# cocowy1/Cost-Volume-Aggregation-in-Stereo-Matching-Revisited

Hardware: AMD Instinct MI355X
Metric: cost-volumes/sec (fwd+bwd) at 544x960 D=192 (higher is better)
Workload: dtype f32

## Files before the change

### cost-volume-aggregation-in-stereo-matching-revisited_amd/csrc/conv3d_wgrad_s2_f16x2.hip

```cpp
#include "dca_frag.h"
#include <type_traits>

namespace {

constexpr int NT = 2;
constexpr int TH = 4, TW = 16;
constexpr int NROW = TH;
constexpr int FD = 3, FH = 2 * TH + 1, NFROW = FD * FH;
constexpr int FV = 2 * TW + 1;
constexpr int VB = 64;
constexpr int X_TERM = NFROW * FV * VB;
constexpr int Y_BLK = NROW * TW * VB;
constexpr int Y_TERM = 2 * Y_BLK;
constexpr int X_OFF = 0, Y_OFF = NT * X_TERM;
constexpr int LDS_BYTES = Y_OFF + NT * Y_TERM;
constexpr int NXQ = NFROW * 8 * 4;
constexpr int KXQ = (NXQ + 511) / 512;
constexpr int NXE = NFROW * 4;
constexpr int NYQ = 2 * NROW * 4 * 4;
static_assert(NXQ - 512 + NYQ <= 512, "coarse items fit behind the second round of fine items");

struct WS2Args {
  const float* x;
  const float* dy;
  float* part;
  int N, Cx, Cy, D, H, W;
  int Do, Ho, Wo;
  int nTD, nTH, nTW, nCxT, nCyP;
  const int* xexps;
  const int* yexps;
};

__global__ __launch_bounds__(512) void wgrad3s2_f16x2_kernel(WS2Args a) {
  extern __shared__ __attribute__((aligned(16))) char smem[];
  const int tid = threadIdx.x, lane = tid & 63, wv = tid >> 6, l31 = lane & 31, half = lane >> 5;
  const int blk = wv >> 2, wq = wv & 3;
  const int ct = blockIdx.y, cyp = ct / a.nCxT, cx0 = (ct % a.nCxT) * 32, cy0 = cyp * 64;
  const bool blk_on = cy0 + 32 * blk < a.Cy;

  const long T = (long)a.N * a.nTD * a.nTH * a.nTW;
  const int nx = gridDim.x >= 8 ? 8 : 1, xcd = blockIdx.x % nx;
  const int cnt = (gridDim.x - xcd + nx - 1) / nx;
  const int t_begin = (int)(T * xcd / nx) + blockIdx.x / nx, t_end = (int)(T * (xcd + 1) / nx), t_step = cnt;

  f32x16 acc[7];
#pragma unroll
  for (int j = 0; j < 7; ++j)
#pragma unroll
    for (int r = 0; r < 16; ++r) acc[j][r] = 0.f;

  const int cstride = a.D * a.H * a.W, ystride = a.Do * a.Ho * a.Wo;
  const long xsample = (long)a.Cx * cstride, ysample = (long)a.Cy * ystride;

  const int q4 = (lane & 15) >> 2, chb = (16 * ((lane >> 4) & 1) + 4 * (lane & 3)) * 2;
  const int lane_off_x = (2 * (8 * half + q4)) * VB + chb;
  const int lane_off_y = (8 * half + q4) * VB + chb;

  float4 rq[KXQ][8];
  float re[8];
  int* ex_lds = (int*)(smem + LDS_BYTES);
  if (tid < 32) ex_lds[tid] = (cx0 + tid < a.Cx) ? dca_coherent_loadi(a.xexps + cx0 + tid) : 0;
  else if (tid < 96) ex_lds[tid] = (cy0 + tid - 32 < a.Cy) ? dca_coherent_loadi(a.yexps + cy0 + tid - 32) : 0;
  __syncthreads();
  const int yu = tid - (NXQ - 512);
  auto decode = [&](int tile, int& n, int& d0, int& h0, int& w0) __attribute__((always_inline)) {
    const int tw = tile % a.nTW; tile /= a.nTW;
    const int th = tile % a.nTH; tile /= a.nTH;
    const int td = tile % a.nTD;
    n = tile / a.nTD;
    d0 = td; h0 = th * TH; w0 = tw * TW;
  };
  auto load_tile = [&](int n, int d0, int h0, int w0, int part = -1) __attribute__((always_inline)) {
    const __amdgpu_buffer_rsrc_t xr = dca_rsrc(a.x + (long)n * xsample, xsample * 4);
    const __amdgpu_buffer_rsrc_t yr = dca_rsrc(a.dy + (long)n * ysample, ysample * 4);
#pragma unroll
    for (int k = 0; k < KXQ; ++k) {
      if ((part == 0 && k >= 1) || (part == 1 && k < 1)) continue;
      const int it = tid + 512 * k, cg = it & 3, quad = (it >> 2) & 7, frow = it >> 5;
      const int d = 2 * d0 - 1 + frow / FH, h = 2 * h0 - 1 + frow % FH, w = 2 * w0 + 4 * quad, c0 = cx0 + cg * 8;
      const int ok = (int)(it < NXQ) & (int)((unsigned)d < (unsigned)a.D) & (int)((unsigned)h < (unsigned)a.H) & (int)(w + 3 < a.W);
      const int off = (c0 * cstride + (d * a.H + h) * a.W + w) * 4;
      if (512 * k + (tid & ~63) < NXQ) {
#pragma unroll
        for (int j = 0; j < 8; ++j) rq[k][j] = dca_bload4(xr, off + j * cstride * 4, ok & (int)(c0 + j < a.Cx));
      }
    }
    if (part == 0) return;
    if ((tid & ~63) < NXE + 63) {
      const int cg = tid & 3, frow = tid >> 2, c0 = cx0 + cg * 8;
      const int d = 2 * d0 - 1 + frow / FH, h = 2 * h0 - 1 + frow % FH, w = 2 * w0 - 1;
      const int ok = (int)(tid < NXE) & (int)((unsigned)d < (unsigned)a.D) & (int)((unsigned)h < (unsigned)a.H) &
                     (int)((unsigned)w < (unsigned)a.W);
      const int off = (c0 * cstride + (d * a.H + h) * a.W + w) * 4;
#pragma unroll
      for (int j = 0; j < 8; ++j) re[j] = dca_bload1(xr, off + j * cstride * 4, ok & (int)(c0 + j < a.Cx));
    }
    if ((unsigned)yu < (unsigned)NYQ) {
      const int cg = yu & 3, quad = (yu >> 2) & 3, row = (yu >> 4) & 3, by = yu >> 6;
      const int h = h0 + row, w = w0 + 4 * quad, c0 = cy0 + 32 * by + cg * 8;
      const int ok = (int)(h < a.Ho) & (int)(w + 3 < a.Wo);
      const int off = (c0 * ystride + (d0 * a.Ho + h) * a.Wo + w) * 4;
#pragma unroll
      for (int j = 0; j < 8; ++j) rq[1][j] = dca_bload4(yr, off + j * ystride * 4, ok & (int)(c0 + j < a.Cy));
    }
  };
  auto split_word = [&](const float (&v)[8], const int* exp8, char* dst, int term_stride) __attribute__((always_inline)) {
    const int4 e0 = *(const int4*)exp8, e1 = *(const int4*)(exp8 + 4);
    const int ex[8] = {e0.x, e0.y, e0.z, e0.w, e1.x, e1.y, e1.z, e1.w};
    f16x8 hv, lv;
#pragma unroll
    for (int j = 0; j < 8; ++j) {
      _Float16 h, l;
      x2_split(v[j], ex[j], h, l);
      hv[j] = h; lv[j] = l;
    }
    *(f16x8*)dst = hv;
    *(f16x8*)(dst + term_stride) = lv;
  };
  auto quad_words = [&](const float4 (&q)[8], const int* ex, char* dst, int term_stride) __attribute__((always_inline)) {
    const float* q0 = (const float*)&q[0];
#pragma unroll
    for (int vv = 0; vv < 4; ++vv) {
      const float v[8] = {q0[vv], q0[4 + vv], q0[8 + vv], q0[12 + vv], q0[16 + vv], q0[20 + vv], q0[24 + vv], q0[28 + vv]};
      split_word(v, ex, dst + vv * VB, term_stride);
    }
  };
  auto store_tile = [&]() __attribute__((always_inline)) {
#pragma unroll
    for (int k = 0; k < KXQ; ++k) {
      const int it = tid + 512 * k, cg = it & 3, quad = (it >> 2) & 7, frow = it >> 5;
      if (it < NXQ) quad_words(rq[k], ex_lds + cg * 8, smem + X_OFF + (frow * FV + 1 + 4 * quad) * VB + cg * 16, X_TERM);
    }
    if (tid < NXE) {
      const int cg = tid & 3, frow = tid >> 2;
      const float v[8] = {re[0], re[1], re[2], re[3], re[4], re[5], re[6], re[7]};
      split_word(v, ex_lds + cg * 8, smem + X_OFF + (frow * FV) * VB + cg * 16, X_TERM);
    }
    if ((unsigned)yu < (unsigned)NYQ) {
      const int cg = yu & 3, quad = (yu >> 2) & 3, row = (yu >> 4) & 3, by = yu >> 6;
      quad_words(rq[1], ex_lds + 32 + 32 * by + cg * 8, smem + Y_OFF + by * Y_BLK + (row * TW + 4 * quad) * VB + cg * 16, Y_TERM);
    }
  };

  auto mfma_tile = [&](auto WQC, bool more, int next_tile) __attribute__((always_inline)) {
    constexpr int WQ = decltype(WQC)::value;
    constexpr int TAP0 = 7 * WQ, TAP1 = (TAP0 + 7 < 27) ? TAP0 + 7 : 27, NTAP = TAP1 - TAP0;
#pragma unroll 1
    for (int i = 0; i < NROW; ++i) {
      if ((i == 1 || i == 2) && more) {
        int nn, nd0, nh0, nw0;
        decode(next_tile, nn, nd0, nh0, nw0);
        load_tile(nn, nd0, nh0, nw0, i - 1);
      }
      if (blk_on) {
        const char* yb = smem + Y_OFF + blk * Y_BLK + (i * TW) * VB + lane_off_y;
        const char* xb = smem + X_OFF + ((2 * i) * FV) * VB + lane_off_x;
        f16x8 ay[NT];
#pragma unroll
        for (int term = 0; term < NT; ++term) ay[term] = tr_frag(yb + term * Y_TERM, 4 * VB);
        f16x8 bx[2][NT];
        auto load_b = [&](int tap, int slot) __attribute__((always_inline)) {
          const int kd = tap / 9, kh = (tap / 3) % 3, kw = tap % 3;
#pragma unroll
          for (int term = 0; term < NT; ++term)
            bx[slot][term] = tr_frag(xb + term * X_TERM + ((kd * FH + kh) * FV + kw) * VB, 8 * VB);
        };
        load_b(TAP0, 0);
#pragma unroll
        for (int j = 0; j < NTAP; ++j) {
          const int cur = j & 1;
          if (j + 1 < NTAP) load_b(TAP0 + j + 1, cur ^ 1);
          acc[j] = __builtin_amdgcn_mfma_f32_32x32x16_f16(ay[0], bx[cur][1], acc[j], 0, 0, 0);
          acc[j] = __builtin_amdgcn_mfma_f32_32x32x16_f16(ay[1], bx[cur][0], acc[j], 0, 0, 0);
          acc[j] = __builtin_amdgcn_mfma_f32_32x32x16_f16(ay[0], bx[cur][0], acc[j], 0, 0, 0);
          if (j + 1 < NTAP) {
            __builtin_amdgcn_sched_group_barrier(0x100, 2, 0);
            __builtin_amdgcn_sched_group_barrier(0x008, 1, 0);
            __builtin_amdgcn_sched_group_barrier(0x100, 2, 0);
            __builtin_amdgcn_sched_group_barrier(0x008, 2, 0);
          }
          __builtin_amdgcn_sched_barrier(0);
        }
      }
    }
  };

  if (t_begin < t_end) {
    int n, d0, h0, w0;
    decode(t_begin, n, d0, h0, w0);
    load_tile(n, d0, h0, w0);
    store_tile();
    __syncthreads();
#pragma unroll 1
    for (int tile = t_begin; tile < t_end; tile += t_step) {
      const bool more = tile + t_step < t_end;
      switch (wq) {
        case 0: mfma_tile(std::integral_constant<int, 0>{}, more, tile + t_step); break;
        case 1: mfma_tile(std::integral_constant<int, 1>{}, more, tile + t_step); break;
        case 2: mfma_tile(std::integral_constant<int, 2>{}, more, tile + t_step); break;
        default: mfma_tile(std::integral_constant<int, 3>{}, more, tile + t_step); break;
      }
      __syncthreads();
      if (more) store_tile();
      __syncthreads();
    }
  }

  if (blk_on) {
    const int xe_l = ex_lds[l31];
    int ninv[16];
#pragma unroll
    for (int r = 0; r < 16; ++r) ninv[r] = -(ex_lds[32 + 32 * blk + (r & 3) + 8 * (r >> 2) + 4 * half] + xe_l);
    const int nCT32 = a.nCxT * ((a.Cy + 31) / 32), ct32 = (2 * cyp + blk) * a.nCxT + (ct % a.nCxT);
    float* slab = a.part + ((long)blockIdx.x * nCT32 + ct32) * 27 * 1024;
#pragma unroll
    for (int j = 0; j < 7; ++j) {
      const int tap = 7 * wq + j;
      if (tap < 27) {
#pragma unroll
        for (int r = 0; r < 16; ++r) {
          const int co = (r & 3) + 8 * (r >> 2) + 4 * half;
          slab[tap * 1024 + co * 32 + l31] = ldexpf(acc[j][r], ninv[r]);
        }
      }
    }
  }
}

struct WS2Geom {
  int Do, Ho, Wo, nTD, nTH, nTW, nCxT, nCyP, nWG, nCT, nblk;
  long ntiles, part_floats;
};
WS2Geom ws2_geometry(int N, int Cx, int Cy, int D, int H, int W) {
  WS2Geom g;
  g.Do = (D + 1) / 2; g.Ho = (H + 1) / 2; g.Wo = (W + 1) / 2;
  g.nTD = g.Do; g.nTH = cdiv(g.Ho, TH); g.nTW = cdiv(g.Wo, TW);
  g.ntiles = (long)N * g.nTD * g.nTH * g.nTW;
  g.nCxT = cdiv(Cx, 32); g.nCyP = cdiv(Cy, 64);
  g.nWG = g.nCxT * g.nCyP;
  g.nCT = g.nCxT * cdiv(Cy, 32);
  g.nblk = dca_persistent_grid(g.ntiles, g.nWG);
  g.part_floats = (long)g.nblk * g.nCT * 27 * 1024;
  return g;
}

}

extern "C" long dca_conv3d_wgrad_s2_x2_workspace(int N, int Cx, int Cy, int D, int H, int W) {
  if (N <= 0 || Cx <= 0 || Cy <= 0 || D <= 0 || H <= 0 || W <= 0) return 0;
  return ws2_geometry(N, Cx, Cy, D, H, W).part_floats;
}

extern "C" int dca_conv3d_wgrad_s2_x2(const float* f, const int* f_exps, const float* c, const int* c_exps,
                                      float* part, float* dw, int N, int Cx, int Cy, int D, int H, int W, long s_cy,
                                      long s_cx, hipStream_t stream) {
  DCA_REQUIRE(f && c && part && dw && f_exps && c_exps && N > 0 && Cx > 0 && Cy > 0 && D > 0 && H > 0 && W > 0);
// ... 18 lines not shown
```

### cost-volume-aggregation-in-stereo-matching-revisited_amd/csrc/pointwise.hip

```cpp
#include "dca_frag.h"
#include "../../include/dca_hip.h"

__global__ __launch_bounds__(256) void bn_stats_kernel(const float* __restrict__ x, double* __restrict__ part, int N,
                                                       int C, long S, int nchunk, long chunk_len, int vec) {
  const int c = blockIdx.x, ch = blockIdx.y, tid = threadIdx.x;
  const long s0 = ch * chunk_len, s1 = min(S, s0 + chunk_len);
  const float K = x[(long)c * S];
  if (ch == 0 && tid == 0) part[(long)C * nchunk * 2 + c] = (double)K;
  float s = 0.f, ss = 0.f;
  for (int n = 0; n < N; ++n) {
    const float* p = x + ((long)n * C + c) * S;
    if (vec) {
      for (long i = s0 + 4 * tid; i < s1; i += 1024) {
        float4 v = *(const float4*)(p + i);
        v.x -= K; v.y -= K; v.z -= K; v.w -= K;
        s += (v.x + v.y) + (v.z + v.w);
        ss += (v.x * v.x + v.y * v.y) + (v.z * v.z + v.w * v.w);
      }
    } else {
      for (long i = s0 + tid; i < s1; i += 256) {
        const float v = p[i] - K;
        s += v;
        ss += v * v;
      }
// ... 485 lines not shown
  const __amdgpu_buffer_rsrc_t xr = dca_rsrc(x + nc * plane, plane * 4);
  const int HW = Ho * Wo, end = min(HW, ((int)blockIdx.y + 1) * 1024);
  for (int i = blockIdx.y * 1024 + threadIdx.x; i < end; i += 256) {
    const int oh = i / Wo, ow = i - oh * Wo;
    float s = 0.f;
#pragma unroll
    for (int kd = 0; kd < 3; ++kd) {
      const int d = 2 * od - 1 + kd;
#pragma unroll
      for (int kh = 0; kh < 3; ++kh) {
        const int h = 2 * oh - 1 + kh;
#pragma unroll
        for (int kw = 0; kw < 3; ++kw) {
          const int w = 2 * ow - 1 + kw;
          const int ok = (int)((unsigned)d < (unsigned)Di) & (int)((unsigned)h < (unsigned)Hi) & (int)((unsigned)w < (unsigned)Wi);
          s += dca_bload1(xr, ((d * Hi + h) * Wi + w) * 4, ok);
        }
      }
    }
    y[row * HW + i] = s * (1.0f / 27.0f);
  }
}

__global__ __launch_bounds__(256) void avgpool3d_bwd_kernel(const float* __restrict__ gy, float* __restrict__ gx,
                                                            const float* __restrict__ res, const float* __restrict__ res2,
                                                            int Di, int Hi, int Wi, int Do, int Ho, int Wo) {
  const long row = blockIdx.x;
  const int d = (int)(row % Di);
  const long nc = row / Di;
  const long plane = (long)Do * Ho * Wo;
  const __amdgpu_buffer_rsrc_t gr = dca_rsrc(gy + nc * plane, plane * 4);
  const int HW = Hi * Wi, end = min(HW, ((int)blockIdx.y + 1) * 1024);
  const int d0 = d >> 1, dn = d & 1;
  for (int i = blockIdx.y * 1024 + threadIdx.x; i < end; i += 256) {
    const int h = i / Wi, w = i - h * Wi;
    const int h0 = h >> 1, hn = h & 1, w0 = w >> 1, wn = w & 1;
    float s = 0.f;
#pragma unroll
    for (int a = 0; a < 2; ++a)
#pragma unroll
      for (int b = 0; b < 2; ++b)
#pragma unroll
        for (int c = 0; c < 2; ++c) {
          const int od = d0 + a, oh = h0 + b, ow = w0 + c;
          const int ok = (a <= dn) & (b <= hn) & (c <= wn) & (int)(od < Do) & (int)(oh < Ho) & (int)(ow < Wo);
          s += dca_bload1(gr, ((od * Ho + oh) * Wo + ow) * 4, ok);
        }
    float o = s * (1.0f / 27.0f) + (res ? res[row * HW + i] : 0.f);
    if (res2) o += res2[row * HW + i];
    gx[row * HW + i] = o;
  }
}

__global__ __launch_bounds__(256) void avgpool3d_fwd_tiled_kernel(const float* __restrict__ x, float* __restrict__ y,
                                                                  int Di, int Hi, int Wi, int Do, int Ho, int Wo) {
  constexpr int TH = 8, TW = 32, FH = 2 * TH + 1, PW = 2 * TW + 2;
  __shared__ __attribute__((aligned(16))) float tile[3 * FH * PW];
  const int tid = threadIdx.x, ow0 = blockIdx.x * TW, oh0 = blockIdx.y * TH;
  const int od = blockIdx.z % Do;
  const long nc = blockIdx.z / Do;
  const long plane = (long)Di * Hi * Wi;
  const __amdgpu_buffer_rsrc_t xr = dca_rsrc(x + nc * plane, plane * 4);
  constexpr int NQ = 3 * FH * 16, KQ = (NQ + 255) / 256;
  float4 rq[KQ];
#pragma unroll
  for (int k = 0; k < KQ; ++k) {
    const int it = tid + 256 * k, q = it & 15, row = it >> 4, a = row / FH, b = row - a * FH;
    const int d = 2 * od - 1 + a, h = 2 * oh0 - 1 + b, w = 2 * ow0 + 4 * q;
    const int ok = (int)(it < NQ) & (int)((unsigned)d < (unsigned)Di) & (int)((unsigned)h < (unsigned)Hi) & (int)(w < Wi);
    rq[k] = dca_bload4(xr, ((d * Hi + h) * Wi + w) * 4, ok);
  }
  float redge = 0.f;
  {
    const int a = tid / FH, b = tid - a * FH;
    const int d = 2 * od - 1 + a, h = 2 * oh0 - 1 + b, w = 2 * ow0 - 1;
    const int ok = (int)(tid < 3 * FH) & (int)((unsigned)d < (unsigned)Di) & (int)((unsigned)h < (unsigned)Hi) &
                   (int)((unsigned)w < (unsigned)Wi);
    redge = dca_bload1(xr, ((d * Hi + h) * Wi + w) * 4, ok);
  }
#pragma unroll
  for (int k = 0; k < KQ; ++k) {
    const int it = tid + 256 * k;
    if (it < NQ) {
      float* p = tile + (it >> 4) * PW + 1 + 4 * (it & 15);
      p[0] = rq[k].x; p[1] = rq[k].y; p[2] = rq[k].z; p[3] = rq[k].w;
    }
  }
  if (tid < 3 * FH) tile[tid * PW] = redge;
  __syncthreads();
  const int hl = tid >> 5, wl = tid & 31, oh = oh0 + hl, ow = ow0 + wl;
  if (oh >= Ho || ow >= Wo) return;
  float s = 0.f;
#pragma unroll
  for (int kd = 0; kd < 3; ++kd)
#pragma unroll
    for (int kh = 0; kh < 3; ++kh) {
      const float* row = tile + (kd * FH + 2 * hl + kh) * PW + 2 * wl;
      const float2 lo = *(const float2*)row;
      s += lo.x;
      s += lo.y;
      s += row[2];
    }
  y[((nc * Do + od) * Ho + oh) * (long)Wo + ow] = s * (1.0f / 27.0f);
}

__global__ __launch_bounds__(256) void avgpool3d_bwd_vec_kernel(const float* __restrict__ gy, float* __restrict__ gx,
                                                                const float* __restrict__ res, const float* __restrict__ res2,
                                                                int Di, int Hi, int Wi, int Do, int Ho, int Wo) {
  const int BD = Di / 2 + 1, BH = Hi / 2 + 1;
  const int bd = (int)(blockIdx.x % BD);
  const long nc = blockIdx.x / BD;
  const long plane = (long)Do * Ho * Wo;
  const __amdgpu_buffer_rsrc_t gr = dca_rsrc(gy + nc * plane, plane * 4);
  const int WQ = Wi >> 2, HQ = BH * WQ, end = min(HQ, ((int)blockIdx.y + 1) * 1024);
  for (int i = blockIdx.y * 1024 + threadIdx.x; i < end; i += 256) {
    const int bh = i / WQ, t = i - bh * WQ, c0 = 2 * t;
    float g[2][2][3];
#pragma unroll
    for (int a = 0; a < 2; ++a)
#pragma unroll
      for (int b = 0; b < 2; ++b)
#pragma unroll
        for (int c = 0; c < 3; ++c) {
          const int od = bd - 1 + a, oh = bh - 1 + b, ow = c0 + c;
          const int ok = (int)((unsigned)od < (unsigned)Do) & (int)((unsigned)oh < (unsigned)Ho) & (int)(ow < Wo);
          g[a][b][c] = dca_bload1(gr, ((od * Ho + oh) * Wo + ow) * 4, ok);
        }
#pragma unroll
    for (int pd = 0; pd < 2; ++pd) {
      const int d = 2 * bd - 1 + pd;
      if ((unsigned)d >= (unsigned)Di) continue;
#pragma unroll
      for (int ph = 0; ph < 2; ++ph) {
        const int h = 2 * bh - 1 + ph;
        if ((unsigned)h >= (unsigned)Hi) continue;
        float o[4];
#pragma unroll
        for (int e = 0; e < 4; ++e) {
          float s = 0.f;
#pragma unroll
          for (int a = pd; a < 2; ++a)
#pragma unroll
            for (int b = ph; b < 2; ++b) {
              s += g[a][b][e >> 1];
              s += (e & 1) ? g[a][b][(e + 1) >> 1] : 0.f;
            }
          o[e] = s * (1.0f / 27.0f);
        }
        const long off = ((nc * Di + d) * Hi + h) * (long)Wi + 4 * t;
        if (res) {
          const float4 r = *(const float4*)(res + off);
          o[0] += r.x; o[1] += r.y; o[2] += r.z; o[3] += r.w;
        }
        if (res2) {
          const float4 r = *(const float4*)(res2 + off);
          o[0] += r.x; o[1] += r.y; o[2] += r.z; o[3] += r.w;
// ... 105 lines not shown
#pragma unroll
  for (int pd = 0; pd < 2; ++pd)
#pragma unroll
    for (int ph = 0; ph < 2; ++ph) {
      const int a0 = pd ? 1 : 0, a1 = pd ? 2 : 1, b0 = ph ? 1 : 0, b1 = ph ? 2 : 1;
      const float wa0 = pd ? 0.75f : 0.25f, wa1 = pd ? 0.25f : 0.75f, wb0 = ph ? 0.75f : 0.25f, wb1 = ph ? 0.25f : 0.75f;
      float2 o;
      o.x = wa0 * (wb0 * r0[a0][b0] + wb1 * r0[a0][b1]) + wa1 * (wb0 * r0[a1][b0] + wb1 * r0[a1][b1]);
      o.y = wa0 * (wb0 * r1[a0][b0] + wb1 * r1[a0][b1]) + wa1 * (wb0 * r1[a1][b0] + wb1 * r1[a1][b1]);
      *(float2*)(q + ((long)(2 * md + pd) * Ho + 2 * mh + ph) * Wo + 2 * mw) = o;
    }
}

__device__ __forceinline__ void up2_bwd_w(int i, int n, float w[4]) {
  w[0] = (i > 0) ? 0.25f : 0.f;
  w[1] = (i > 0) ? 0.75f : 1.0f;
  w[2] = (i < n - 1) ? 0.75f : 1.0f;
  w[3] = (i < n - 1) ? 0.25f : 0.f;
}

__global__ __launch_bounds__(256) void trilinear_up2_bwd_kernel(const float* __restrict__ gy, float* __restrict__ gx,
                                                                int Di, int Hi, int Wi) {
  const int w = blockIdx.x * 256 + threadIdx.x, h = blockIdx.y;
  const int d = blockIdx.z % Di;
  const long nc = blockIdx.z / Di;
  const int Ho = 2 * Hi, Wo = 2 * Wi;
  const long plane = (2L * Di) * Ho * Wo;
  const __amdgpu_buffer_rsrc_t gr = dca_rsrc(gy + nc * plane, plane * 4);
  const int wok = (int)(w < Wi);
  float wd[4], wh[4], ww[4];
  up2_bwd_w(d, Di, wd); up2_bwd_w(h, Hi, wh); up2_bwd_w(w, Wi, ww);
  float acc = 0.f;
#pragma unroll
  for (int a = 0; a < 4; ++a) {
    const int od = 2 * d - 1 + a;
#pragma unroll
    for (int b = 0; b < 4; ++b) {
      const int oh = 2 * h - 1 + b;
      const int ok = wok & (int)(wd[a] != 0.f) & (int)(wh[b] != 0.f);
      const int off = ((od * Ho + oh) * Wo + 2 * w) * 4;
      const float2 mid = dca_bload2(gr, off, ok);
      const float lo = dca_bload1(gr, off - 4, ok & (int)(ww[0] != 0.f));
      const float hi = dca_bload1(gr, off + 8, ok & (int)(ww[3] != 0.f));
      float r = ww[1] * mid.x + ww[2] * mid.y;
      r += ww[0] * lo;
      r += ww[3] * hi;
      acc += wd[a] * wh[b] * r;
    }
  }
  if (wok) gx[((nc * Di + d) * Hi + h) * Wi + w] = acc;
}

__global__ __launch_bounds__(256) void trilinear_up2_bwd_tiled_kernel(const float* __restrict__ gy, float* __restrict__ gx,
                                                                      int Di, int Hi, int Wi) {
  constexpr int TH = 8, TW = 32, FH = 2 * TH + 2, FW = 2 * TW + 2, PW = FW + 2;
  __shared__ __attribute__((aligned(16))) float tile[4 * FH * PW];
  const int tid = threadIdx.x, w0 = blockIdx.x * TW, h0 = blockIdx.y * TH;
  const int d = blockIdx.z % Di;
  const long nc = blockIdx.z / Di;
  const int Do = 2 * Di, Ho = 2 * Hi, Wo = 2 * Wi;
  const long plane = (long)Do * Ho * Wo;
  const __amdgpu_buffer_rsrc_t gr = dca_rsrc(gy + nc * plane, plane * 4);
  constexpr int NQ = 4 * FH * 16, KQ = (NQ + 255) / 256;
  float4 rq[KQ];
#pragma unroll
  for (int k = 0; k < KQ; ++k) {
    const int it = tid + 256 * k, q = it & 15, row = it >> 4, a = row / FH, b = row - a * FH;
    const int od = 2 * d - 1 + a, oh = 2 * h0 - 1 + b, ow = 2 * w0 + 4 * q;
    const int ok = (int)(it < NQ) & (int)((unsigned)od < (unsigned)Do) & (int)((unsigned)oh < (unsigned)Ho) &
                   (int)(ow < Wo);
    rq[k] = dca_bload4(gr, ((od * Ho + oh) * Wo + ow) * 4, ok);
  }
  float redge = 0.f;
  {
    const int side = tid & 1, row = tid >> 1, a = row / FH, b = row - a * FH;
    const int od = 2 * d - 1 + a, oh = 2 * h0 - 1 + b, ow = side ? 2 * w0 + 2 * TW : 2 * w0 - 1;
    const int ok = (int)(tid < 4 * FH * 2) & (int)((unsigned)od < (unsigned)Do) & (int)((unsigned)oh < (unsigned)Ho) &
                   (int)((unsigned)ow < (unsigned)Wo);
    redge = dca_bload1(gr, ((od * Ho + oh) * Wo + ow) * 4, ok);
  }
#pragma unroll
  for (int k = 0; k < KQ; ++k) {
    const int it = tid + 256 * k;
    if (it < NQ) {
      float* p = tile + (it >> 4) * PW + 1 + 4 * (it & 15);
      p[0] = rq[k].x; p[1] = rq[k].y; p[2] = rq[k].z; p[3] = rq[k].w;
    }
  }
  if (tid < 4 * FH * 2) tile[(tid >> 1) * PW + ((tid & 1) ? FW - 1 : 0)] = redge;
  __syncthreads();
  const int hl = tid >> 5, wl = tid & 31, h = h0 + hl, w = w0 + wl;
  if (h >= Hi || w >= Wi) return;
  float wd[4], wh[4], ww[4];
  up2_bwd_w(d, Di, wd); up2_bwd_w(h, Hi, wh); up2_bwd_w(w, Wi, ww);
  float acc = 0.f;
#pragma unroll
  for (int a = 0; a < 4; ++a)
#pragma unroll
    for (int b = 0; b < 4; ++b) {
      const float* row = tile + (a * FH + 2 * hl + b) * PW + 2 * wl;
      const float2 lo = *(const float2*)row, hi = *(const float2*)(row + 2);
      float r = ww[1] * lo.y + ww[2] * hi.x;
      r += ww[0] * lo.x;
      r += ww[3] * hi.y;
      acc += wd[a] * wh[b] * r;
    }
  gx[((nc * Di + d) * Hi + h) * Wi + w] = acc;
}

static int ew_grid(long total) {
  long g = (total + 255) / 256;
  return (int)(g < 8192 ? (g > 0 ? g : 1) : 8192);
}

static void chunking(long S, int C, int* nchunk, long* chunk_len) {
  long want = (2048 + C - 1) / C;
  if (want > 256) want = 256;
  long len = (S + want - 1) / want;
  len = ((len + 1023) / 1024) * 1024;
  *chunk_len = len;
  *nchunk = (int)((S + len - 1) / len);
}

extern "C" int dca_bn_num_chunks(int C, long S) {
  int n; long l;
  chunking(S, C, &n, &l);
  return n;
}
extern "C" int dca_bn_pack_chunks(int C, long S) {
  int n; long l;
  chunking(S, (C + 7) / 8, &n, &l);
  return n;
}

extern "C" int dca_bn_stats(const float* x, double* part, int N, int C, long S, hipStream_t stream) {
  DCA_REQUIRE(x && part && N > 0 && C > 0 && S > 0 && C <= 65535);
  int nchunk; long len;
  chunking(S, C, &nchunk, &len);
  const int vec = (S % 4 == 0) && (((uintptr_t)x & 15) == 0);
  hipLaunchKernelGGL(bn_stats_kernel, dim3(C, nchunk), dim3(256), 0, stream, x, part, N, C, S, nchunk, len, vec);
  return dca_launch_status();
}

extern "C" int dca_bn_finalize(const double* part, int nchunk, double count, const float* gamma, const float* beta,
                               float* running_mean, float* running_var, float momentum, float eps, int training,
                               float* stats, int* zexps, const unsigned* rpre_slots, int rpre_n,
                               const unsigned* rpost_slots, int rpost_n, int C, hipStream_t stream) {
  DCA_REQUIRE(stats && C > 0 && (training ? (part != nullptr && nchunk > 0) : (running_mean && running_var)));
  DCA_REQUIRE(zexps == nullptr || training);
  DCA_REQUIRE((rpre_slots == nullptr || (rpre_n > 0 && rpre_n <= DCA_AMAX_CSLOTS)) &&
              (rpost_slots == nullptr || (rpost_n > 0 && rpost_n <= DCA_AMAX_CSLOTS)));
  hipLaunchKernelGGL(bn_finalize_kernel, dim3(C), dim3(64), 0, stream, part, nchunk, count, gamma, beta,
                     running_mean, running_var, momentum, eps, training, stats, zexps, rpre_slots, rpre_n, rpost_slots,
                     rpost_n, C);
  return dca_launch_status();
}

extern "C" int dca_bn_finalize_centered(const double* part, int nchunk, const float* gamma, const float* beta,
                                        float* running_mean, float* running_var, float momentum, float eps, float* stats,
                                        int* zexps, const unsigned* rpre_slots, int rpre_n, const unsigned* rpost_slots,
// ... 40 lines not shown
  const int vec = (S % 4 == 0) && ((((uintptr_t)x) & 15) == 0);
  hipLaunchKernelGGL(cmax_kernel, dim3(nchunk, C), dim3(256), 0, stream, x, N, C, S, len, vec, slots);
  return dca_launch_status();
}

extern "C" int dca_cmax_exps(const unsigned* slots, int nslots, int C, int* exps, hipStream_t stream) {
  DCA_REQUIRE(slots && exps && C > 0 && nslots > 0 && nslots <= DCA_AMAX_CSLOTS);
  hipLaunchKernelGGL(cmax_exps_kernel, dim3(C), dim3(64), 0, stream, slots, nslots, exps);
  return dca_launch_status();
}

extern "C" int dca_bn_backward(const float* dz, const float* y, const float* res_pre, const float* stats,
                               double* part, float* dgb, float* dy, float* g_out, int N, int C, long S, float slope,
                               int training, unsigned* dmax, hipStream_t stream) {
  DCA_REQUIRE(dz && y && stats && part && dgb && dy && N > 0 && C > 0 && S > 0 && C <= 65535);
  int nchunk; long len;
  chunking(S, C, &nchunk, &len);
  const uintptr_t al = (uintptr_t)dz | (uintptr_t)y | (uintptr_t)res_pre | (uintptr_t)dy | (uintptr_t)g_out;
  const int vec = (S % 4 == 0) && ((al & 15) == 0);
  hipLaunchKernelGGL(bn_bwd_reduce_kernel, dim3(C, nchunk), dim3(256), 0, stream, dz, y, res_pre, stats, part, N, C, S,
                     nchunk, len, slope, vec, (unsigned*)nullptr);
  hipLaunchKernelGGL(bn_bwd_finalize_kernel, dim3(C), dim3(64), 0, stream, part, nchunk, (double)N * (double)S, dgb, C,
                     stats, training, (const unsigned*)nullptr, (const unsigned*)nullptr, 0, (int*)nullptr);
  hipLaunchKernelGGL(bn_bwd_apply_kernel, dim3(nchunk, C), dim3(256), 0, stream, dz, y, res_pre, stats, dgb, dy, g_out, N, C,
                     S, len, slope, training, vec, dmax);
  return dca_launch_status();
}

extern "C" int dca_bn_backward_pack(const float* dz, const float* y, const float* stats, double* part, float* dgb, void* dyp,
                                    int* dyexps, unsigned* gmax, const unsigned* ymax, int ymax_slots, int N, int C, long S,
                                    float slope, int training, hipStream_t stream) {
  DCA_REQUIRE(dz && y && stats && part && dgb && dyp && dyexps && gmax && N > 0 && C > 0 && C % 8 == 0 && S > 0 && C <= 65535);
  DCA_REQUIRE((ymax == nullptr || (ymax_slots > 0 && ymax_slots <= DCA_AMAX_CSLOTS)) && ((((uintptr_t)dyp) & 15) == 0));
  int nchunk; long len;
  chunking(S, C, &nchunk, &len);
  const uintptr_t al = (uintptr_t)dz | (uintptr_t)y;
  const int vec = (S % 4 == 0) && ((al & 15) == 0);
  hipLaunchKernelGGL(bn_bwd_reduce_kernel, dim3(C, nchunk), dim3(256), 0, stream, dz, y, (const float*)nullptr, stats, part,
                     N, C, S, nchunk, len, slope, vec, gmax);
  hipLaunchKernelGGL(bn_bwd_finalize_kernel, dim3(C), dim3(64), 0, stream, part, nchunk, (double)N * (double)S, dgb, C,
                     stats, training, (const unsigned*)gmax, ymax, ymax_slots, dyexps);
  int pchunk; long plen;
  chunking(S, C / 8, &pchunk, &plen);
  hipLaunchKernelGGL(bn_bwd_apply_pack_kernel, dim3(pchunk, C / 8), dim3(256), 0, stream, dz, y, stats, dgb, dyexps,
                     (char*)dyp, N, C, S, plen, slope, training);
  return dca_launch_status();
}

extern "C" int dca_avgpool3d_fwd(const float* x, float* y, long NC, int Di, int Hi, int Wi, hipStream_t stream) {
  DCA_REQUIRE(x && y && NC > 0 && Di > 0 && Hi > 0 && Wi > 0);
  const int Do = (Di + 1) / 2, Ho = (Hi + 1) / 2, Wo = (Wi + 1) / 2;
  DCA_REQUIRE((long)Di * Hi * Wi * 4 < 0x7ffffff0L && NC * Do < 0x7fffffffL);
  if (Wi % 4 == 0 && (((uintptr_t)x) & 15) == 0 && NC * Do <= 65535 && cdiv(Ho, 8) <= 65535) {
    hipLaunchKernelGGL(avgpool3d_fwd_tiled_kernel, dim3(cdiv(Wo, 32), cdiv(Ho, 8), (unsigned)(NC * Do)), dim3(256), 0, stream,
                       x, y, Di, Hi, Wi, Do, Ho, Wo);
    return dca_launch_status();
  }
  hipLaunchKernelGGL(avgpool3d_fwd_kernel, dim3((unsigned)(NC * Do), cdiv((long)Ho * Wo, 1024)), dim3(256), 0, stream, x,
                     y, Di, Hi, Wi, Do, Ho, Wo);
  return dca_launch_status();
}

extern "C" int dca_avgpool3d_bwd(const float* gy, float* gx, const float* res, const float* res2, long NC, int Di, int Hi,
                                 int Wi, hipStream_t stream) {
  DCA_REQUIRE(gy && gx && NC > 0 && Di > 0 && Hi > 0 && Wi > 0 && (res || !res2));
  const int Do = (Di + 1) / 2, Ho = (Hi + 1) / 2, Wo = (Wi + 1) / 2;
  DCA_REQUIRE((long)Di * Hi * Wi * 4 < 0x7ffffff0L && NC * Di < 0x7fffffffL);
  if (Wi % 4 == 0 && ((((uintptr_t)gx) | ((uintptr_t)res) | ((uintptr_t)res2)) & 15) == 0) {
    hipLaunchKernelGGL(avgpool3d_bwd_vec_kernel, dim3((unsigned)(NC * (Di / 2 + 1)), cdiv((long)(Hi / 2 + 1) * (Wi / 4), 1024)),
                       dim3(256), 0, stream, gy, gx, res, res2, Di, Hi, Wi, Do, Ho, Wo);
    return dca_launch_status();
  }
  hipLaunchKernelGGL(avgpool3d_bwd_kernel, dim3((unsigned)(NC * Di), cdiv((long)Hi * Wi, 1024)), dim3(256), 0, stream, gy,
                     gx, res, res2, Di, Hi, Wi, Do, Ho, Wo);
  return dca_launch_status();
}

extern "C" int dca_trilinear_fwd(const float* x, float* y, long NC, int Di, int Hi, int Wi, int scale,
                                 hipStream_t stream) {
  DCA_REQUIRE(x && y && NC > 0 && Di > 0 && Hi > 0 && Wi > 0 && scale >= 1);
  if (scale == 2 && Hi <= 65535 && NC * Di <= 65535 && (((uintptr_t)y & 7) == 0)) {
    hipLaunchKernelGGL(trilinear_up2_fwd_kernel, dim3(cdiv(Wi, 64), cdiv(Hi, 4), (unsigned)(NC * Di)), dim3(256), 0, stream,
                       x, y, Di, Hi, Wi);
    return dca_launch_status();
  }
  const long total = NC * Di * Hi * Wi * scale * scale * scale;
  hipLaunchKernelGGL(trilinear_fwd_kernel, dim3(ew_grid(total)), dim3(256), 0, stream, x, y, NC, Di, Hi, Wi, scale);
  return dca_launch_status();
}

extern "C" int dca_trilinear_bwd(const float* gy, float* gx, long NC, int Di, int Hi, int Wi, int scale,
                                 hipStream_t stream) {
  DCA_REQUIRE(gy && gx && NC > 0 && Di > 0 && Hi > 0 && Wi > 0 && scale >= 1);
  if (scale == 2 && cdiv(Hi, 8) <= 65535 && NC * Di <= 65535 && 32L * Di * Hi * Wi < 0x7ffffff0L && Wi % 2 == 0 &&
      (((uintptr_t)gy & 15) == 0)) {
    hipLaunchKernelGGL(trilinear_up2_bwd_tiled_kernel, dim3(cdiv(Wi, 32), cdiv(Hi, 8), (unsigned)(NC * Di)), dim3(256), 0,
                       stream, gy, gx, Di, Hi, Wi);
    return dca_launch_status();
  }
  if (scale == 2 && Hi <= 65535 && NC * Di <= 65535 && 32L * Di * Hi * Wi < 0x7ffffff0L && (((uintptr_t)gy & 7) == 0)) {
    hipLaunchKernelGGL(trilinear_up2_bwd_kernel, dim3(cdiv(Wi, 256), Hi, (unsigned)(NC * Di)), dim3(256), 0, stream, gy, gx,
                       Di, Hi, Wi);
    return dca_launch_status();
  }
  hipLaunchKernelGGL(trilinear_bwd_kernel, dim3(ew_grid(NC * Di * Hi * Wi)), dim3(256), 0, stream, gy, gx, NC, Di, Hi,
                     Wi, scale);
  return dca_launch_status();
}
```

Measured before the change: 39.39.

## Reuse overlapping depth planes via LDS ring buffers in strided wgrad, avgpool, upsample-bwd

The stride-2 weight-gradient conv kernel now gives each block a contiguous run of tiles ordered depth-fastest. The input halo planes are kept in a 3-slot ring in shared memory, so consecutive depth tiles load only the two new planes instead of all three. The XCD-interleaved tile schedule is dropped in favour of that contiguous split. The avgpool3d forward and trilinear up2 backward tiled kernels now loop over segments of eight output depths per block with a similar ring buffer, which cuts redundant global reads of the overlapping planes at the cost of fewer blocks and more per-block serialization.

Result: no change. 39.39 (-0.0%).

```diff
diff --git a/cost-volume-aggregation-in-stereo-matching-revisited_amd/csrc/conv3d_wgrad_s2_f16x2.hip b/cost-volume-aggregation-in-stereo-matching-revisited_amd/csrc/conv3d_wgrad_s2_f16x2.hip
--- a/cost-volume-aggregation-in-stereo-matching-revisited_amd/csrc/conv3d_wgrad_s2_f16x2.hip
+++ b/cost-volume-aggregation-in-stereo-matching-revisited_amd/csrc/conv3d_wgrad_s2_f16x2.hip
@@ -39,9 +39,7 @@
   const bool blk_on = cy0 + 32 * blk < a.Cy;
 
   const long T = (long)a.N * a.nTD * a.nTH * a.nTW;
-  const int nx = gridDim.x >= 8 ? 8 : 1, xcd = blockIdx.x % nx;
-  const int cnt = (gridDim.x - xcd + nx - 1) / nx;
-  const int t_begin = (int)(T * xcd / nx) + blockIdx.x / nx, t_end = (int)(T * (xcd + 1) / nx), t_step = cnt;
+  const int t_begin = (int)(T * blockIdx.x / gridDim.x), t_end = (int)(T * (blockIdx.x + 1) / gridDim.x);
 
   f32x16 acc[7];
 #pragma unroll
@@ -64,32 +62,33 @@
   __syncthreads();
   const int yu = tid - (NXQ - 512);
   auto decode = [&](int tile, int& n, int& d0, int& h0, int& w0) __attribute__((always_inline)) {
+    const int td = tile % a.nTD; tile /= a.nTD;
     const int tw = tile % a.nTW; tile /= a.nTW;
-    const int th = tile % a.nTH; tile /= a.nTH;
-    const int td = tile % a.nTD;
-    n = tile / a.nTD;
+    const int th = tile % a.nTH;
+    n = tile / a.nTH;
     d0 = td; h0 = th * TH; w0 = tw * TW;
   };
-  auto load_tile = [&](int n, int d0, int h0, int w0, int part = -1) __attribute__((always_inline)) {
+  auto load_tile = [&](int n, int d0, int h0, int w0, bool march, int part = -1) __attribute__((always_inline)) {
     const __amdgpu_buffer_rsrc_t xr = dca_rsrc(a.x + (long)n * xsample, xsample * 4);
     const __amdgpu_buffer_rsrc_t yr = dca_rsrc(a.dy + (long)n * ysample, ysample * 4);
+    const int fr0 = march ? FH : 0, nxq = NXQ - 32 * fr0, nxe = NXE - 4 * fr0;
 #pragma unroll
     for (int k = 0; k < KXQ; ++k) {
       if ((part == 0 && k >= 1) || (part == 1 && k < 1)) continue;
-      const int it = tid + 512 * k, cg = it & 3, quad = (it >> 2) & 7, frow = it >> 5;
+      const int it = tid + 512 * k, cg = it & 3, quad = (it >> 2) & 7, frow = fr0 + (it >> 5);
       const int d = 2 * d0 - 1 + frow / FH, h = 2 * h0 - 1 + frow % FH, w = 2 * w0 + 4 * quad, c0 = cx0 + cg * 8;
-      const int ok = (int)(it < NXQ) & (int)((unsigned)d < (unsigned)a.D) & (int)((unsigned)h < (unsigned)a.H) & (int)(w + 3 < a.W);
+      const int ok = (int)(it < nxq) & (int)((unsigned)d < (unsigned)a.D) & (int)((unsigned)h < (unsigned)a.H) & (int)(w + 3 < a.W);
       const int off = (c0 * cstride + (d * a.H + h) * a.W + w) * 4;
-      if (512 * k + (tid & ~63) < NXQ) {
+      if (512 * k + (tid & ~63) < nxq) {
 #pragma unroll
         for (int j = 0; j < 8; ++j) rq[k][j] = dca_bload4(xr, off + j * cstride * 4, ok & (int)(c0 + j < a.Cx));
       }
     }
     if (part == 0) return;
-    if ((tid & ~63) < NXE + 63) {
-      const int cg = tid & 3, frow = tid >> 2, c0 = cx0 + cg * 8;
+    if ((tid & ~63) < nxe) {
+      const int cg = tid & 3, frow = fr0 + (tid >> 2), c0 = cx0 + cg * 8;
       const int d = 2 * d0 - 1 + frow / FH, h = 2 * h0 - 1 + frow % FH, w = 2 * w0 - 1;
-      const int ok = (int)(tid < NXE) & (int)((unsigned)d < (unsigned)a.D) & (int)((unsigned)h < (unsigned)a.H) &
+      const int ok = (int)(tid < nxe) & (int)((unsigned)d < (unsigned)a.D) & (int)((unsigned)h < (unsigned)a.H) &
                      (int)((unsigned)w < (unsigned)a.W);
       const int off = (c0 * cstride + (d * a.H + h) * a.W + w) * 4;
 #pragma unroll
@@ -125,16 +124,21 @@
       split_word(v, ex, dst + vv * VB, term_stride);
     }
   };
-  auto store_tile = [&]() __attribute__((always_inline)) {
+  auto ring_row = [&](int d0, int frow) __attribute__((always_inline)) {
+    const int kd = frow / FH;
+    return ((2 * d0 + kd) % 3) * FH + (frow - kd * FH);
+  };
+  auto store_tile = [&](int d0, bool march) __attribute__((always_inline)) {
+    const int fr0 = march ? FH : 0, nxq = NXQ - 32 * fr0, nxe = NXE - 4 * fr0;
 #pragma unroll
     for (int k = 0; k < KXQ; ++k) {
-      const int it = tid + 512 * k, cg = it & 3, quad = (it >> 2) & 7, frow = it >> 5;
-      if (it < NXQ) quad_words(rq[k], ex_lds + cg * 8, smem + X_OFF + (frow * FV + 1 + 4 * quad) * VB + cg * 16, X_TERM);
-    }
-    if (tid < NXE) {
-      const int cg = tid & 3, frow = tid >> 2;
+      const int it = tid + 512 * k, cg = it & 3, quad = (it >> 2) & 7, row = ring_row(d0, fr0 + (it >> 5));
+      if (it < nxq) quad_words(rq[k], ex_lds + cg * 8, smem + X_OFF + (row * FV + 1 + 4 * quad) * VB + cg * 16, X_TERM);
+    }
+    if (tid < nxe) {
+      const int cg = tid & 3, row = ring_row(d0, fr0 + (tid >> 2));
       const float v[8] = {re[0], re[1], re[2], re[3], re[4], re[5], re[6], re[7]};
-      split_word(v, ex_lds + cg * 8, smem + X_OFF + (frow * FV) * VB + cg * 16, X_TERM);
+      split_word(v, ex_lds + cg * 8, smem + X_OFF + (row * FV) * VB + cg * 16, X_TERM);
     }
     if ((unsigned)yu < (unsigned)NYQ) {
       const int cg = yu & 3, quad = (yu >> 2) & 3, row = (yu >> 4) & 3, by = yu >> 6;
@@ -142,15 +146,16 @@
     }
   };
 
-  auto mfma_tile = [&](auto WQC, bool more, int next_tile) __attribute__((always_inline)) {
+  auto mfma_tile = [&](auto WQC, int d0, bool more, int next_tile) __attribute__((always_inline)) {
     constexpr int WQ = decltype(WQC)::value;
     constexpr int TAP0 = 7 * WQ, TAP1 = (TAP0 + 7 < 27) ? TAP0 + 7 : 27, NTAP = TAP1 - TAP0;
+    const int xslot[3] = {ring_row(d0, 0) * FV * VB, ring_row(d0, FH) * FV * VB, ring_row(d0, 2 * FH) * FV * VB};
 #pragma unroll 1
     for (int i = 0; i < NROW; ++i) {
       if ((i == 1 || i == 2) && more) {
         int nn, nd0, nh0, nw0;
         decode(next_tile, nn, nd0, nh0, nw0);
-        load_tile(nn, nd0, nh0, nw0, i - 1);
+        load_tile(nn, nd0, nh0, nw0, nd0 != 0, i - 1);
       }
       if (blk_on) {
         const char* yb = smem + Y_OFF + blk * Y_BLK + (i * TW) * VB + lane_off_y;
@@ -163,7 +168,7 @@
           const int kd = tap / 9, kh = (tap / 3) % 3, kw = tap % 3;
 #pragma unroll
           for (int term = 0; term < NT; ++term)
-            bx[slot][term] = tr_frag(xb + term * X_TERM + ((kd * FH + kh) * FV + kw) * VB, 8 * VB);
+            bx[slot][term] = tr_frag(xb + xslot[kd] + term * X_TERM + (kh * FV + kw) * VB, 8 * VB);
         };
         load_b(TAP0, 0);
 #pragma unroll
@@ -188,20 +193,21 @@
   if (t_begin < t_end) {
     int n, d0, h0, w0;
     decode(t_begin, n, d0, h0, w0);
-    load_tile(n, d0, h0, w0);
-    store_tile();
+    load_tile(n, d0, h0, w0, false);
+    store_tile(d0, false);
     __syncthreads();
 #pragma unroll 1
-    for (int tile = t_begin; tile < t_end; tile += t_step) {
-      const bool more = tile + t_step < t_end;
+    for (int tile = t_begin; tile < t_end; ++tile) {
+      const bool more = tile + 1 < t_end;
+      const int td = tile % a.nTD, ntd = td + 1 < a.nTD ? td + 1 : 0;
       switch (wq) {
-        case 0: mfma_tile(std::integral_constant<int, 0>{}, more, tile + t_step); break;
-        case 1: mfma_tile(std::integral_constant<int, 1>{}, more, tile + t_step); break;
-        case 2: mfma_tile(std::integral_constant<int, 2>{}, more, tile + t_step); break;
-        default: mfma_tile(std::integral_constant<int, 3>{}, more, tile + t_step); break;
+        case 0: mfma_tile(std::integral_constant<int, 0>{}, td, more, tile + 1); break;
+        case 1: mfma_tile(std::integral_constant<int, 1>{}, td, more, tile + 1); break;
+        case 2: mfma_tile(std::integral_constant<int, 2>{}, td, more, tile + 1); break;
+        default: mfma_tile(std::integral_constant<int, 3>{}, td, more, tile + 1); break;
       }
       __syncthreads();
-      if (more) store_tile();
+      if (more) store_tile(ntd, ntd != 0);
       __syncthreads();
     }
   }
diff --git a/cost-volume-aggregation-in-stereo-matching-revisited_amd/csrc/pointwise.hip b/cost-volume-aggregation-in-stereo-matching-revisited_amd/csrc/pointwise.hip
--- a/cost-volume-aggregation-in-stereo-matching-revisited_amd/csrc/pointwise.hip
+++ b/cost-volume-aggregation-in-stereo-matching-revisited_amd/csrc/pointwise.hip
@@ -561,56 +561,76 @@
   }
 }
 
+constexpr int DEPTH_SEG = 8;
 __global__ __launch_bounds__(256) void avgpool3d_fwd_tiled_kernel(const float* __restrict__ x, float* __restrict__ y,
-                                                                  int Di, int Hi, int Wi, int Do, int Ho, int Wo) {
+                                                                  int Di, int Hi, int Wi, int Do, int Ho, int Wo, int nseg) {
   constexpr int TH = 8, TW = 32, FH = 2 * TH + 1, PW = 2 * TW + 2;
+  constexpr int PQ = FH * 16;
   __shared__ __attribute__((aligned(16))) float tile[3 * FH * PW];
   const int tid = threadIdx.x, ow0 = blockIdx.x * TW, oh0 = blockIdx.y * TH;
-  const int od = blockIdx.z % Do;
-  const long nc = blockIdx.z / Do;
+  const int od_begin = (int)(blockIdx.z % nseg) * DEPTH_SEG, od_end = min(Do, od_begin + DEPTH_SEG);
+  const long nc = blockIdx.z / nseg;
   const long plane = (long)Di * Hi * Wi;
   const __amdgpu_buffer_rsrc_t xr = dca_rsrc(x + nc * plane, plane * 4);
-  constexpr int NQ = 3 * FH * 16, KQ = (NQ + 255) / 256;
-  float4 rq[KQ];
-#pragma unroll
-  for (int k = 0; k < KQ; ++k) {
-    const int it = tid + 256 * k, q = it & 15, row = it >> 4, a = row / FH, b = row - a * FH;
-    const int d = 2 * od - 1 + a, h = 2 * oh0 - 1 + b, w = 2 * ow0 + 4 * q;
-    const int ok = (int)(it < NQ) & (int)((unsigned)d < (unsigned)Di) & (int)((unsigned)h < (unsigned)Hi) & (int)(w < Wi);
-    rq[k] = dca_bload4(xr, ((d * Hi + h) * Wi + w) * 4, ok);
-  }
+  float4 rq[(3 * PQ + 255) / 256];
   float redge = 0.f;
-  {
+  auto load = [&](auto NPC, int p0) __attribute__((always_inline)) {
+    constexpr int NP = decltype(NPC)::value, NQ = NP * PQ, KQ = (NQ + 255) / 256;
+#pragma unroll
+    for (int k = 0; k < KQ; ++k) {
+      const int it = tid + 256 * k, q = it & 15, row = it >> 4, a = row / FH, b = row - a * FH;
+      const int d = p0 + a, h = 2 * oh0 - 1 + b, w = 2 * ow0 + 4 * q;
+      const int ok = (int)(it < NQ) & (int)((unsigned)d < (unsigned)Di) & (int)((unsigned)h < (unsigned)Hi) & (int)(w < Wi);
+      rq[k] = dca_bload4(xr, ((d * Hi + h) * Wi + w) * 4, ok);
+    }
     const int a = tid / FH, b = tid - a * FH;
-    const int d = 2 * od - 1 + a, h = 2 * oh0 - 1 + b, w = 2 * ow0 - 1;
-    const int ok = (int)(tid < 3 * FH) & (int)((unsigned)d < (unsigned)Di) & (int)((unsigned)h < (unsigned)Hi) &
+    const int d = p0 + a, h = 2 * oh0 - 1 + b, w = 2 * ow0 - 1;
+    const int ok = (int)(tid < NP * FH) & (int)((unsigned)d < (unsigned)Di) & (int)((unsigned)h < (unsigned)Hi) &
                    (int)((unsigned)w < (unsigned)Wi);
     redge = dca_bload1(xr, ((d * Hi + h) * Wi + w) * 4, ok);
-  }
-#pragma unroll
-  for (int k = 0; k < KQ; ++k) {
-    const int it = tid + 256 * k;
-    if (it < NQ) {
-      float* p = tile + (it >> 4) * PW + 1 + 4 * (it & 15);
-      p[0] = rq[k].x; p[1] = rq[k].y; p[2] = rq[k].z; p[3] = rq[k].w;
-    }
-  }
-  if (tid < 3 * FH) tile[tid * PW] = redge;
+  };
+  auto store = [&](auto NPC, int p0) __attribute__((always_inline)) {
+    constexpr int NP = decltype(NPC)::value, NQ = NP * PQ, KQ = (NQ + 255) / 256;
+#pragma unroll
+    for (int k = 0; k < KQ; ++k) {
+      const int it = tid + 256 * k, row = it >> 4, a = row / FH, b = row - a * FH;
+      if (it < NQ) {
+        float* p = tile + (((p0 + a + 1) % 3) * FH + b) * PW + 1 + 4 * (it & 15);
+        p[0] = rq[k].x; p[1] = rq[k].y; p[2] = rq[k].z; p[3] = rq[k].w;
+      }
+    }
+    if (tid < NP * FH) tile[(((p0 + tid / FH + 1) % 3) * FH + tid % FH) * PW] = redge;
+  };
+  const std::integral_constant<int, 3> three;
+  const std::integral_constant<int, 2> two;
+  load(three, 2 * od_begin - 1);
+  store(three, 2 * od_begin - 1);
   __syncthreads();
   const int hl = tid >> 5, wl = tid & 31, oh = oh0 + hl, ow = ow0 + wl;
-  if (oh >= Ho || ow >= Wo) return;
-  float s = 0.f;
-#pragma unroll
-  for (int kd = 0; kd < 3; ++kd)
-#pragma unroll
-    for (int kh = 0; kh < 3; ++kh) {
-      const float* row = tile + (kd * FH + 2 * hl + kh) * PW + 2 * wl;
-      const float2 lo = *(const float2*)row;
-      s += lo.x;
-      s += lo.y;
-      s += row[2];
-    }
-  y[((nc * Do + od) * Ho + oh) * (long)Wo + ow] = s * (1.0f / 27.0f);
+  const bool live = oh < Ho && ow < Wo;
+  for (int od = od_begin; od < od_end; ++od) {
+    const bool more = od + 1 < od_end;
+    if (more) load(two, 2 * od + 2);
+    if (live) {
+      float s = 0.f;
+#pragma unroll
+      for (int kd = 0; kd < 3; ++kd)
+#pragma unroll
+        for (int kh = 0; kh < 3; ++kh) {
+          const float* row = tile + (((2 * od + kd) % 3) * FH + 2 * hl + kh) * PW + 2 * wl;
+          const float2 lo = *(const float2*)row;
+          s += lo.x;
+          s += lo.y;
+          s += row[2];
+        }
+      y[((nc * Do + od) * Ho + oh) * (long)Wo + ow] = s * (1.0f / 27.0f);
+    }
+    if (more) {
+      __syncthreads();
+      store(two, 2 * od + 2);
+      __syncthreads();
+    }
+  }
 }
 
 __global__ __launch_bounds__(256) void avgpool3d_bwd_vec_kernel(const float* __restrict__ gy, float* __restrict__ gx,
@@ -822,60 +842,84 @@
 }
 
 __global__ __launch_bounds__(256) void trilinear_up2_bwd_tiled_kernel(const float* __restrict__ gy, float* __restrict__ gx,
-                                                                      int Di, int Hi, int Wi) {
+                                                                      int Di, int Hi, int Wi, int nseg) {
   constexpr int TH = 8, TW = 32, FH = 2 * TH + 2, FW = 2 * TW + 2, PW = FW + 2;
+  constexpr int PQ = FH * 16;
   __shared__ __attribute__((aligned(16))) float tile[4 * FH * PW];
   const int tid = threadIdx.x, w0 = blockIdx.x * TW, h0 = blockIdx.y * TH;
-  const int d = blockIdx.z % Di;
-  const long nc = blockIdx.z / Di;
+  const int d_begin = (int)(blockIdx.z % nseg) * DEPTH_SEG, d_end = min(Di, d_begin + DEPTH_SEG);
+  const long nc = blockIdx.z / nseg;
   const int Do = 2 * Di, Ho = 2 * Hi, Wo = 2 * Wi;
   const long plane = (long)Do * Ho * Wo;
   const __amdgpu_buffer_rsrc_t gr = dca_rsrc(gy + nc * plane, plane * 4);
-  constexpr int NQ = 4 * FH * 16, KQ = (NQ + 255) / 256;
-  float4 rq[KQ];
-#pragma unroll
-  for (int k = 0; k < KQ; ++k) {
-    const int it = tid + 256 * k, q = it & 15, row = it >> 4, a = row / FH, b = row - a * FH;
-    const int od = 2 * d - 1 + a, oh = 2 * h0 - 1 + b, ow = 2 * w0 + 4 * q;
-    const int ok = (int)(it < NQ) & (int)((unsigned)od < (unsigned)Do) & (int)((unsigned)oh < (unsigned)Ho) &
-                   (int)(ow < Wo);
-    rq[k] = dca_bload4(gr, ((od * Ho + oh) * Wo + ow) * 4, ok);
-  }
+  float4 rq[(4 * PQ + 255) / 256];
   float redge = 0.f;
-  {
+  auto load = [&](auto NPC, int p0) __attribute__((always_inline)) {
+    constexpr int NP = decltype(NPC)::value, NQ = NP * PQ, KQ = (NQ + 255) / 256;
+#pragma unroll
+    for (int k = 0; k < KQ; ++k) {
+      const int it = tid + 256 * k, q = it & 15, row = it >> 4, a = row / FH, b = row - a * FH;
+      const int od = p0 + a, oh = 2 * h0 - 1 + b, ow = 2 * w0 + 4 * q;
+      const int ok = (int)(it < NQ) & (int)((unsigned)od < (unsigned)Do) & (int)((unsigned)oh < (unsigned)Ho) &
+                     (int)(ow < Wo);
+      rq[k] = dca_bload4(gr, ((od * Ho + oh) * Wo + ow) * 4, ok);
+    }
     const int side = tid & 1, row = tid >> 1, a = row / FH, b = row - a * FH;
-    const int od = 2 * d - 1 + a, oh = 2 * h0 - 1 + b, ow = side ? 2 * w0 + 2 * TW : 2 * w0 - 1;
-    const int ok = (int)(tid < 4 * FH * 2) & (int)((unsigned)od < (unsigned)Do) & (int)((unsigned)oh < (unsigned)Ho) &
+    const int od = p0 + a, oh = 2 * h0 - 1 + b, ow = side ? 2 * w0 + 2 * TW : 2 * w0 - 1;
+    const int ok = (int)(tid < NP * FH * 2) & (int)((unsigned)od < (unsigned)Do) & (int)((unsigned)oh < (unsigned)Ho) &
                    (int)((unsigned)ow < (unsigned)Wo);
     redge = dca_bload1(gr, ((od * Ho + oh) * Wo + ow) * 4, ok);
-  }
-#pragma unroll
-  for (int k = 0; k < KQ; ++k) {
-    const int it = tid + 256 * k;
-    if (it < NQ) {
-      float* p = tile + (it >> 4) * PW + 1 + 4 * (it & 15);
-      p[0] = rq[k].x; p[1] = rq[k].y; p[2] = rq[k].z; p[3] = rq[k].w;
-    }
-  }
-  if (tid < 4 * FH * 2) tile[(tid >> 1) * PW + ((tid & 1) ? FW - 1 : 0)] = redge;
+  };
+  auto store = [&](auto NPC, int p0) __attribute__((always_inline)) {
+    constexpr int NP = decltype(NPC)::value, NQ = NP * PQ, KQ = (NQ + 255) / 256;
+#pragma unroll
+    for (int k = 0; k < KQ; ++k) {
+      const int it = tid + 256 * k, row = it >> 4, a = row / FH, b = row - a * FH;
+      if (it < NQ) {
+        float* p = tile + (((p0 + a + 1) & 3) * FH + b) * PW + 1 + 4 * (it & 15);
+        p[0] = rq[k].x; p[1] = rq[k].y; p[2] = rq[k].z; p[3] = rq[k].w;
+      }
+    }
+    if (tid < NP * FH * 2) {
+      const int row = tid >> 1, a = row / FH, b = row - a * FH;
+      tile[(((p0 + a + 1) & 3) * FH + b) * PW + ((tid & 1) ? FW - 1 : 0)] = redge;
+    }
+  };
+  const std::integral_constant<int, 4> four;
+  const std::integral_constant<int, 2> two;
+  load(four, 2 * d_begin - 1);
+  store(four, 2 * d_begin - 1);
   __syncthreads();
   const int hl = tid >> 5, wl = tid & 31, h = h0 + hl, w = w0 + wl;
-  if (h >= Hi || w >= Wi) return;
-  float wd[4], wh[4], ww[4];
-  up2_bwd_w(d, Di, wd); up2_bwd_w(h, Hi, wh); up2_bwd_w(w, Wi, ww);
-  float acc = 0.f;
-#pragma unroll
-  for (int a = 0; a < 4; ++a)
-#pragma unroll
-    for (int b = 0; b < 4; ++b) {
-      const float* row = tile + (a * FH + 2 * hl + b) * PW + 2 * wl;
-      const float2 lo = *(const float2*)row, hi = *(const float2*)(row + 2);
-      float r = ww[1] * lo.y + ww[2] * hi.x;
-      r += ww[0] * lo.x;
-      r += ww[3] * hi.y;
-      acc += wd[a] * wh[b] * r;
-    }
-  gx[((nc * Di + d) * Hi + h) * Wi + w] = acc;
+  const bool live = h < Hi && w < Wi;
+  float wh[4], ww[4];
+  up2_bwd_w(h, Hi, wh); up2_bwd_w(w, Wi, ww);
+  for (int d = d_begin; d < d_end; ++d) {
+    const bool more = d + 1 < d_end;
+    if (more) load(two, 2 * d + 3);
+    if (live) {
+      float wd[4];
+      up2_bwd_w(d, Di, wd);
+      float acc = 0.f;
+#pragma unroll
+      for (int a = 0; a < 4; ++a)
+#pragma unroll
+        for (int b = 0; b < 4; ++b) {
+          const float* row = tile + (((2 * d + a) & 3) * FH + 2 * hl + b) * PW + 2 * wl;
+          const float2 lo = *(const float2*)row, hi = *(const float2*)(row + 2);
+          float r = ww[1] * lo.y + ww[2] * hi.x;
+          r += ww[0] * lo.x;
+          r += ww[3] * hi.y;
+          acc += wd[a] * wh[b] * r;
+        }
+      gx[((nc * Di + d) * Hi + h) * Wi + w] = acc;
+    }
+    if (more) {
+      __syncthreads();
+      store(two, 2 * d + 3);
+      __syncthreads();
+    }
+  }
 }
 
 static int ew_grid(long total) {
@@ -1022,8 +1066,9 @@
   const int Do = (Di + 1) / 2, Ho = (Hi + 1) / 2, Wo = (Wi + 1) / 2;
   DCA_REQUIRE((long)Di * Hi * Wi * 4 < 0x7ffffff0L && NC * Do < 0x7fffffffL);
   if (Wi % 4 == 0 && (((uintptr_t)x) & 15) == 0 && NC * Do <= 65535 && cdiv(Ho, 8) <= 65535) {
-    hipLaunchKernelGGL(avgpool3d_fwd_tiled_kernel, dim3(cdiv(Wo, 32), cdiv(Ho, 8), (unsigned)(NC * Do)), dim3(256), 0, stream,
-                       x, y, Di, Hi, Wi, Do, Ho, Wo);
+    const int nseg = cdiv(Do, DEPTH_SEG);
+    hipLaunchKernelGGL(avgpool3d_fwd_tiled_kernel, dim3(cdiv(Wo, 32), cdiv(Ho, 8), (unsigned)(NC * nseg)), dim3(256), 0, stream,
+                       x, y, Di, Hi, Wi, Do, Ho, Wo, nseg);
     return dca_launch_status();
   }
   hipLaunchKernelGGL(avgpool3d_fwd_kernel, dim3((unsigned)(NC * Do), cdiv((long)Ho * Wo, 1024)), dim3(256), 0, stream, x,
@@ -1064,8 +1109,9 @@
   DCA_REQUIRE(gy && gx && NC > 0 && Di > 0 && Hi > 0 && Wi > 0 && scale >= 1);
   if (scale == 2 && cdiv(Hi, 8) <= 65535 && NC * Di <= 65535 && 32L * Di * Hi * Wi < 0x7ffffff0L && Wi % 2 == 0 &&
       (((uintptr_t)gy & 15) == 0)) {
-    hipLaunchKernelGGL(trilinear_up2_bwd_tiled_kernel, dim3(cdiv(Wi, 32), cdiv(Hi, 8), (unsigned)(NC * Di)), dim3(256), 0,
-                       stream, gy, gx, Di, Hi, Wi);
+    const int nseg = cdiv(Di, DEPTH_SEG);
+    hipLaunchKernelGGL(trilinear_up2_bwd_tiled_kernel, dim3(cdiv(Wi, 32), cdiv(Hi, 8), (unsigned)(NC * nseg)), dim3(256), 0,
+                       stream, gy, gx, Di, Hi, Wi, nseg);
     return dca_launch_status();
   }
   if (scale == 2 && Hi <= 65535 && NC * Di <= 65535 && 32L * Di * Hi * Wi < 0x7ffffff0L && (((uintptr_t)gy & 7) == 0)) {
```
